# isaac-chandler/cuda-raytracer

Hardware: AMD Instinct MI355X
Metric: Mrays/s (live ray segments/s, teapot) (higher is better)
Workload: dtype f32

## Files before the change

cuda-raytracer_amd/csrc/rt_render.hip:

```cpp
#include "rt_common.h"

#include <algorithm>
#include <chrono>
#include <cstdio>
#include <cstdlib>
#include <cstring>
#include <string>
#include <thread>
#include <vector>

#include <rccl/rccl.h>

#pragma clang fp contract(off)

int rtamd_render_multi(const rt_scene *scene, const rt_opts *opts, float *fb_out, rt_stats *stats);

using namespace rtamd;

namespace {

#ifndef RT_INFLIGHT
#define RT_INFLIGHT 20
#endif
#ifndef RT_TRACE_OCC
// ... 20 lines not shown
    return (n + span - 1) / span;
}
inline int max_tiles(int64_t n_max) {
    return n_max >= (int64_t)kTileTarget * kSortTile ? (int)((n_max + kSortTile - 1) / kSortTile)
                                                    : (int)std::min<int64_t>(kTileTarget, (n_max + kBlock - 1) / kBlock);
}
inline int tile_stride(int64_t n_max) {
    return (int)std::max<int64_t>(kTileTarget, (n_max + kSortTile - 1) / kSortTile);
}
constexpr int kBuckets = 65;
constexpr int kInflight = RT_INFLIGHT;
constexpr int kStaggerUs = 4000;
constexpr int kStaggerGroup = 4;
constexpr int kStaggerMinPasses = 8;
constexpr int kStaggerShortUs = 2000;
constexpr int kTraceOccPct = RT_TRACE_OCC;
constexpr uint32_t kDead = 64;
constexpr uint32_t kAccFlag = 0x80000000u;
constexpr int kSpanSlots = 8;
constexpr int kSpanWords = 2 * kSpanSlots;
#ifdef RT_PROFILE
__device__ unsigned long long g_prof[2][14];
#define PROF(i, v) (prof[i] += (v))
#else
#define PROF(i, v) ((void)0)
#endif

struct FastDiv {
    uint32_t m = 0;
    int l = 0;
    static FastDiv of(uint32_t d) {
        FastDiv f;
        if (d > 1) {
            f.l = 32 - __builtin_clz(d - 1);
            f.m = (uint32_t)((((uint64_t)1 << (31 + f.l)) + d - 1) / d);
        }
        return f;
    }
    __device__ __forceinline__ uint32_t div(uint32_t n) const { return l == 0 ? n : (__umulhi(n, m) >> (l - 1)); }
};

struct SlotMap {
    FastDiv by_stripe;
    uint32_t skip, base;
    static SlotMap identity() { return SlotMap{FastDiv::of(0x7fffffffu), 0u, 0u}; }
    static SlotMap of(uint32_t stripe, int count, int index) {
        return SlotMap{FastDiv::of(stripe), (uint32_t)(count - 1) * stripe, (uint32_t)index * stripe};
    }
    __device__ __forceinline__ uint32_t ray(uint32_t s) const { return s + by_stripe.div(s) * skip + base; }
};

template <int FIRST>
__device__ __forceinline__ uint32_t first_ray(const SlotMap &m, uint32_t slot) {
    return FIRST == 2 ? m.ray(slot) : slot;
}

struct PassArgs {
    int rtc;
    uint32_t gen_seed_term;
    FastDiv by_rtc, by_width;
    SlotMap map;
};

__device__ __forceinline__ V3 primary_dir(const DevScene &S, int i, const PassArgs &pa) {
    Rng rng = pcg_seed((uint32_t)i * 0x85810BEAu + pa.gen_seed_term);
    uint32_t z;
    asm volatile("v_mov_b32 %0, 0" : "=v"(z));
    rng.inc += z;
    const uint32_t pixel = pa.by_rtc.div((uint32_t)i);
    const uint32_t yy = pa.by_width.div(pixel);
    const int x = (int)(pixel - yy * (uint32_t)S.width), y = (int)yy;
    const float xc = (x + random01(rng)) * S.inv_w;
    const float yc = (y + random01(rng)) * S.inv_h;
    return normalise(S.tl + xc * S.sr - yc * S.su);
}

#ifndef RT_FUSED_MAX_TRIS
#define RT_FUSED_MAX_TRIS 4096
#endif
#ifndef RT_SORT_GRID
#define RT_SORT_GRID 0
#endif

template <bool SORTED, bool COUNT, int FIRST>
__global__ __launch_bounds__(kBlock) RT_TRACE_ATTR void trace_kernel(DevScene S, PassArgs pa, const float4 *__restrict__ geo,
                                                       const uint32_t *__restrict__ live_count,
                                                       uint32_t *__restrict__ queue, float2 *__restrict__ hits,
                                                       uint32_t *__restrict__ overflow, Counters *__restrict__ ctr,
                                                       unsigned long long *__restrict__ tspan) {
    __shared__ uint2 stack[(kStackLds + 1) * kBlock];
    const unsigned long long t_start = wall_clock64();
    uint2 *col = stack + threadIdx.x;
    const uint32_t lanes = gridDim.x * kBlock, gl = blockIdx.x * kBlock + threadIdx.x;
    const uint32_t dist_half = lanes * (kStackMax - kStackLds);
    const uint32_t L = __builtin_amdgcn_readfirstlane(*live_count);
    const uint32_t waves = gridDim.x * (kBlock / 64);
    const uint32_t chunk = min((uint32_t)kChunkMax, max((uint32_t)kChunkMin, (L / (4 * waves) + 63) & ~63u));
    uint32_t shard = blockIdx.x % kQueues, tried = 0;
    uint32_t q_next = 0, q_end = 0;
    bool exhausted = false;
    int slot = -1;
    V3 o{0, 0, 0}, d{0, 0, 0};
    float ix = 0, iy = 0, iz = 0, closest = 0;
    bool finite_inv = true;
    bool wave_nonfinite = false;
    int index = -1, sp = 0;
    uint32_t ref = 0;
    int ti = 0, te = 0;
    unsigned pn = 0, iv = 0, tt = 0, nlive = 0;
#ifdef RT_PROFILE
    unsigned long long prof[14] = {0, 0, 0, 0, 0, 0, 0, 0, 0, 0, 0, 0, 0, 0};
#endif
    auto node_step = [&](float4 a, float4 b, float4 c, uint2 kids) -> bool {
        if (COUNT) iv++;
        float t0, t1;
        bool h0, h1;
        slab_pair(a, b, c, o, ix, iy, iz, closest, h0, h1, t0, t1);
        if (__builtin_expect(wave_nonfinite, 0)) {
            float u0, u1;
            const bool g0 = slab(a.x, a.z, b.x, b.z, c.x, c.z, o, ix, iy, iz, closest, u0);
            const bool g1 = slab(a.y, a.w, b.y, b.w, c.y, c.w, o, ix, iy, iz, closest, u1);
            if (!finite_inv) { h0 = g0; h1 = g1; t0 = u0; t1 = u1; }
        }
        const bool both = h0 && h1, any = h0 || h1;
        const bool sel1 = h1 && (!h0 || t0 < t1);
        const uint32_t next_ref = sel1 ? kids.y : kids.x, near_ref = sel1 ? kids.x : kids.y;
        const float next_t = sel1 ? t1 : t0, near_t = sel1 ? t0 : t1;
        col[min(sp, kStackLds) * kBlock] = make_uint2(near_ref, __float_as_uint(near_t));
        if (__builtin_expect(both && sp >= kStackLds, 0)) {
            overflow[(sp - kStackLds) * lanes + gl] = near_ref;
            overflow[dist_half + (sp - kStackLds) * lanes + gl] = __float_as_uint(near_t);
        }
        if (both) sp++;
        ref = any ? next_ref : ref;
        const bool descend = any && !(next_t >= closest);
        bool need = !descend;
        if (descend) {
            if (COUNT) pn++;
            if (ref & kLeaf) {
                leaf_range(S, ref, ti, te);
                need = ti == te;
            }
        }
        return need;
    };
    auto pop_loop = [&](bool need) {
        while (need) {
            PROF(10, 1);
            const bool empty = sp == 0;
            sp = empty ? 0 : sp - 1;
            uint2 e = col[min(sp, kStackLds) * kBlock];
            asm volatile("" : "+v"(e.x), "+v"(e.y));
            if (__builtin_expect(__ballot(sp >= kStackLds) != 0, 0)) {
                if (sp >= kStackLds) {
                    e.x = overflow[(sp - kStackLds) * lanes + gl];
                    e.y = overflow[dist_half + (sp - kStackLds) * lanes + gl];
                }
            }
            const bool take = !empty && !(__uint_as_float(e.y) >= closest);
            slot = empty ? -2 - slot : slot;
            ref = take ? e.x : ref;
            if (COUNT) pn += take ? 1u : 0u;
            const bool leaf = take && (ref & kLeaf);
            if (__builtin_expect(leaf && (ref & kBigLeaf), 0)) {
                leaf_range(S, ref, ti, te);
            } else {
                ti = leaf ? (int)(ref & 0xFFFFFFu) : ti;
                te = leaf ? ti + (int)((ref >> 24) & 0x3Fu) : te;
            }
            need = !empty && (!take || (leaf && ti == te));
        }
    };
    const bool root_internal = !(S.root_ref & kLeaf);
    float4 ra{0, 0, 0, 0}, rb{0, 0, 0, 0}, rc{0, 0, 0, 0};
    uint2 rk{0, 0};
    if (root_internal) {
        const float4 *rr = S.nodes + (size_t)S.root_ref * 4;
        const float4 x0 = rr[0], x1 = rr[1], x2 = rr[2];
        const uint2 k = *reinterpret_cast<const uint2 *>(rr + 3);
#define RT_U(v) __int_as_float(__builtin_amdgcn_readfirstlane(__float_as_int(v)))
        ra = make_float4(RT_U(x0.x), RT_U(x0.y), RT_U(x0.z), RT_U(x0.w));
        rb = make_float4(RT_U(x1.x), RT_U(x1.y), RT_U(x1.z), RT_U(x1.w));
        rc = make_float4(RT_U(x2.x), RT_U(x2.y), RT_U(x2.z), RT_U(x2.w));
#undef RT_U
        rk = make_uint2(__builtin_amdgcn_readfirstlane(k.x), __builtin_amdgcn_readfirstlane(k.y));
    }
    while (true) {
        unsigned long long idle = __ballot(slot < 0);
        if (!exhausted && __popcll(idle) >= (FIRST ? kRefillFirst : kRefill)) {
            PROF(6, 1);
            if (slot <= -2) {
                hits[-2 - slot] = make_float2(closest, __int_as_float(index));
                slot = -1;
            }
            bool fresh = false;
            while (idle && !exhausted) {
                if (q_next >= q_end) {
                    const uint32_t seg_lo = (uint32_t)(((uint64_t)L * shard) / kQueues);
                    const uint32_t seg_hi = (uint32_t)(((uint64_t)L * (shard + 1)) / kQueues);
                    uint32_t c = 0;
                    if (lane_id() == 0) c = atomicAdd(queue + shard * kQueueStride, chunk);
                    c = __builtin_amdgcn_readfirstlane(__shfl(c, 0)) + seg_lo;
                    if (c >= seg_hi) {
                        shard = (shard + 1) % kQueues;
                        if (++tried == kQueues) exhausted = true;
                        continue;
                    }
                    q_next = c;
                    q_end = min(c + chunk, seg_hi);
                }
                const uint32_t avail = q_end - q_next;
                const uint32_t r = rank_below(idle);
                const bool take = slot < 0 && r < avail;
                const unsigned long long took = __ballot(take);
                if (take) { slot = (int)(q_next + r); fresh = true; }
                q_next += (uint32_t)__popcll(took);
                idle &= ~took;
            }
            if (fresh) {
                {
                    nlive++;
                    if (FIRST) {
                        o = S.cam;
                        d = primary_dir(S, (int)first_ray<FIRST>(pa.map, (uint32_t)slot), pa);
                    } else {
                        const float4 *rp = geo + (size_t)slot * 2;
                        const float4 r0 = rp[0];
                        const float2 r1 = *reinterpret_cast<const float2 *>(rp + 1);
                        o = v3(r0.x, r0.y, r0.z);
                        d = v3(r0.w, r1.x, r1.y);
                    }
                    ix = 1 / d.x; iy = 1 / d.y; iz = 1 / d.z;
                    finite_inv = __builtin_isfinite(ix) && __builtin_isfinite(iy) && __builtin_isfinite(iz);

                    closest = 1e30f;
                    index = -1;
                    for (int i = 0; i < S.sphere_count; i++) {
                        const float4 sph = S.spheres[i];
                        float t;
                        if (ray_sphere(o, d, v3(sph.x, sph.y, sph.z), sph.w, closest, t)) { closest = t; index = i; }
                    }
                    ref = S.root_ref;
                    sp = 0;
                    if (COUNT) pn++;
                    ti = te = 0;
                    if (ref & kLeaf) {
                        leaf_range(S, ref, ti, te);
                        if (ti == te) {
                            hits[slot] = make_float2(closest, __int_as_float(index));
                            slot = -1;
                        }
                    }
                }
            }
            wave_nonfinite = __ballot(slot >= 0 && !finite_inv) != 0;
            if (root_internal && __ballot(fresh && slot >= 0)) {
                bool need = false;
                if (fresh && slot >= 0) need = node_step(ra, rb, rc, rk);
                pop_loop(need);
            }
        }
        if (!__ballot(slot >= 0)) {
            if (exhausted) break;
            PROF(7, 1);
            continue;
        }
#ifdef RT_PROFILE
        {
            const unsigned long long act = __ballot(slot >= 0), lf = __ballot(slot >= 0 && ti < te);
            PROF(0, 1); PROF(1, __popcll(act)); PROF(2, __popcll(lf));
            PROF(3, lf != 0); PROF(4, (act & ~lf) != 0);
            const bool mixed = lf != 0 && (act & ~lf) != 0;
            PROF(8, mixed);
            if (mixed) PROF(9, min(__popcll(lf), __popcll(act & ~lf)));
            const uintptr_t ra = slot >= 0 ? (uintptr_t)(ti < te ? S.tris + (size_t)ti * 3 : S.nodes + (size_t)ref * 4) : 0;
            const int first = __builtin_ctzll(act);
            const uintptr_t r0 = ((uintptr_t)__shfl((unsigned)(ra >> 32), first) << 32) | __shfl((unsigned)ra, first);
            const unsigned long long same = __ballot(slot >= 0 && ra == r0);
            PROF(12, same == act);
            PROF(13, 4 * __popcll(same) >= 3 * __popcll(act));
        }
#endif
        if (slot < 0) continue;
        bool need = false;
        const bool in_leaf = ti < te;
        const float4 *rec = in_leaf ? S.tris + (size_t)ti * 3 : S.nodes + (size_t)ref * 4;
        const float4 a = rec[0], b = rec[1], c = rec[2];
        uint2 kids = make_uint2(0, 0);
        if (!in_leaf) kids = *reinterpret_cast<const uint2 *>(rec + 3);
        if (in_leaf) {
            const float4 q0 = a, q1 = b;
            const float q2 = c.x;
            if (COUNT) tt++;
            float t;
            const bool hit =
                ray_triangle_flat(o, d, v3(q0.x, q0.y, q0.z), v3(q0.w, q1.x, q1.y), v3(q1.z, q1.w, q2), closest, t);
            closest = hit ? t : closest;
            index = hit ? S.sphere_count + ti : index;
            need = ++ti == te;
        } else {
            need = node_step(a, b, c, kids);
// ... 499 lines not shown
            if (threadIdx.x < kBuckets) {
                uint32_t s2 = 0;
                for (int k = 0; k < kBlock / 64; k++) { s2 += wcount[k][threadIdx.x]; wcount[k][threadIdx.x] = 0; }
                run[threadIdx.x] += s2;
            }
            __syncthreads();
        }
    }
}
__global__ void delay_kernel(unsigned long long ticks) {
    const unsigned long long t0 = wall_clock64();
    while (wall_clock64() - t0 < ticks) __builtin_amdgcn_s_sleep(127);
}

__global__ void set_count_kernel(uint32_t *__restrict__ dst, uint32_t v, const uint32_t *__restrict__ src) {
    if (threadIdx.x == 0) *dst = src ? *src : v;
}

template <bool SORTED, int FIRST, bool INLINE>
__global__ __launch_bounds__(kBlock) RT_REPLAY_ATTR void sort_scatter_shade_kernel(DevScene S, PassArgs pa,
                                                                    const uint8_t *__restrict__ bkt_in,
                                                                    const float4 *__restrict__ geo_in,
                                                                    const float *__restrict__ tz_in,
                                                                    const uint32_t *__restrict__ rid_in,
                                                                    const float2 *__restrict__ hits, uint32_t seed_term,
                                                                    const uint32_t *__restrict__ live_count, int tiles,
                                                                    const uint32_t *__restrict__ offsets,
                                                                    const uint32_t *__restrict__ totals,
                                                                    float4 *__restrict__ geo_out,
                                                                    float *__restrict__ tz_out,
                                                                    uint32_t *__restrict__ rid_out,
                                                                    float4 *__restrict__ acc = nullptr,
                                                                    uint32_t *__restrict__ home_of = nullptr,
                                                                    uint32_t home_base = 0) {
    const bool homes = FIRST == 1 && home_of != nullptr;
    const int n = (int)*live_count;
    __shared__ uint32_t run[kBuckets];
    __shared__ uint32_t wcount[kBlock / 64][kBuckets];
    const int R = tile_rounds(n), span = kBlock * R;
    for (int tile = blockIdx.x; tile * span < n; tile += gridDim.x) {
        bucket_runs(run, offsets, totals, tiles, tile);
        for (int k = threadIdx.x; k < (kBlock / 64) * kBuckets; k += kBlock) (&wcount[0][0])[k] = 0;
        __syncthreads();
        const int wave = threadIdx.x >> 6;
        const int base = tile * span;
        const int rounds = min(R, (n - base + kBlock - 1) / kBlock);
        for (int r = 0; r < rounds; r++) {
            const int item = base + r * kBlock + threadIdx.x;
            const bool valid = item < n;
            const uint32_t b = valid ? bkt_in[item] : 0u;
            const bool move = valid && b != kDead;
            Shaded sh{};
            if (move) sh = shade_one<SORTED, FIRST, INLINE>(S, pa, item, geo_in, tz_in, rid_in, hits, seed_term);
            const unsigned long long peers = match_bucket(b, valid);
            const uint32_t rank = rank_below(peers);
            if (valid && rank == 0) wcount[wave][b] = (uint32_t)__popcll(peers);
            __syncthreads();
            if (move) {
                uint32_t pos = run[b] + rank;
                for (int k = 0; k < wave; k++) pos += wcount[k][b];
                geo_out[(size_t)pos * 2] = make_float4(sh.no.x, sh.no.y, sh.no.z, sh.nd.x);
                geo_out[(size_t)pos * 2 + 1] = make_float4(sh.nd.y, sh.nd.z, sh.T.x, sh.T.y);
                tz_out[pos] = sh.T.z;
                const uint32_t id = homes ? home_base + pos : sh.ray;
                if (homes) {
                    home_of[item] = id;
                    if (has_radiance(sh.C)) acc[id] = make_float4(sh.T.z, sh.C.x, sh.C.y, sh.C.z);
                }
                rid_out[pos] = id | (has_radiance(sh.C) || sh.acc_holds ? kAccFlag : 0u);
            } else if (homes && valid) {
                home_of[item] = (uint32_t)item;
            }
            __syncthreads();
            if (threadIdx.x < kBuckets) {
                uint32_t s = 0;
                for (int k = 0; k < kBlock / 64; k++) { s += wcount[k][threadIdx.x]; wcount[k][threadIdx.x] = 0; }
                run[threadIdx.x] += s;
            }
            __syncthreads();
        }
    }
}

constexpr int kAccPixels = 64;
template <bool TILED>
__global__ __launch_bounds__(kBlock) void accumulate_kernel(const float4 *__restrict__ tc, int rtc, int pixels,
                                                            float *__restrict__ sums, SlotMap pix,
                                                            const uint32_t *__restrict__ home_of = nullptr) {
    __shared__ float col[kAccPixels * 20 * 3];
    const int p0 = blockIdx.x * kAccPixels;
    const int np = min(kAccPixels, pixels - p0);
    const int n = np * rtc;
    const float4 *src = tc + (size_t)p0 * rtc;
    for (int e = threadIdx.x; e < n; e += kBlock) {
        const float4 c = TILED     ? tc[(size_t)pix.ray((uint32_t)(p0 + e / rtc)) * rtc + e % rtc]
                         : home_of ? tc[home_of[(size_t)p0 * rtc + e]]
                                   : src[e];
        col[e * 3] = c.y;
        col[e * 3 + 1] = c.z;
        col[e * 3 + 2] = c.w;
    }
    __syncthreads();
    const int t = threadIdx.x;
    if (t >= np) return;
    float sx = 0, sy = 0, sz = 0;
    const float *r = col + t * rtc * 3;
    for (int s = 0; s < rtc; s++) {
        sx = sx + r[s * 3];
        sy = sy + r[s * 3 + 1];
        sz = sz + r[s * 3 + 2];
    }
    const size_t p = TILED ? (size_t)pix.ray((uint32_t)(p0 + t)) : (size_t)(p0 + t);
    sums[p * 3] = sx;
    sums[p * 3 + 1] = sy;
    sums[p * 3 + 2] = sz;
}

__global__ __launch_bounds__(kBlock) void high_pass_kernel(const float *__restrict__ img, float *__restrict__ out,
                                                           float threshold, int pixels) {
    const int i = blockIdx.x * kBlock + threadIdx.x;
    if (i >= pixels) return;
    const V3 c = v3(img[3 * i], img[3 * i + 1], img[3 * i + 2]);
    const bool bright = dot(c, v3(0.2126f, 0.7152f, 0.0722f)) > threshold;
    out[3 * i] = bright ? c.x : 0.0f;
    out[3 * i + 1] = bright ? c.y : 0.0f;
    out[3 * i + 2] = bright ? c.z : 0.0f;
}

template <bool VERTICAL>
__global__ __launch_bounds__(kBlock) void box_blur_kernel(const float *__restrict__ in, float *__restrict__ out,
                                                          int radius, int w, int h) {
    const int i = blockIdx.x * kBlock + threadIdx.x;
    if (i >= w * h) return;
    const int x = i % w, y = i / w;
    float sx = 0, sy = 0, sz = 0;
    int count = 0;
    for (int k = -radius; k <= radius; k++) {
        const int nx = VERTICAL ? x : x + k, ny = VERTICAL ? y + k : y;
        if (VERTICAL ? (ny >= 0 && ny < h) : (nx >= 0 && nx < w)) {
            const float *p = in + ((size_t)ny * w + nx) * 3;
            sx = sx + p[0];
            sy = sy + p[1];
            sz = sz + p[2];
            count++;
        }
    }
    const float k = 1.0f / count;
    out[3 * i] = k * sx;
    out[3 * i + 1] = k * sy;
    out[3 * i + 2] = k * sz;
}

__global__ __launch_bounds__(kBlock) void add_kernel(float *__restrict__ img, const float *__restrict__ add, int n) {
    const int i = blockIdx.x * kBlock + threadIdx.x;
    if (i < n) img[i] = img[i] + add[i];
}
__global__ __launch_bounds__(kBlock) void add4_kernel(float *__restrict__ img, const float *__restrict__ add, int n) {
    const int i = blockIdx.x * kBlock + threadIdx.x;
    const int n4 = n >> 2;
    if (i < n4) {
        float4 a = reinterpret_cast<float4 *>(img)[i];
        const float4 b = reinterpret_cast<const float4 *>(add)[i];
        a.x = a.x + b.x; a.y = a.y + b.y; a.z = a.z + b.z; a.w = a.w + b.w;
        reinterpret_cast<float4 *>(img)[i] = a;
    }
    if (i < (n & 3)) img[(n4 << 2) + i] = img[(n4 << 2) + i] + add[(n4 << 2) + i];
}

__attribute__((constructor(101))) void rtamd_default_hw_queues() {
    setenv("GPU_MAX_HW_QUEUES", "24", 0);
}
int queues_granted() {
    const char *q = std::getenv("GPU_MAX_HW_QUEUES");
    const int n = q ? std::atoi(q) : 0;
    return n > 0 ? n : 4;
}

}

int rtamd::trace_closest_blocks_per_cu(int &per_cu) {
    HIPCHK(hipOccupancyMaxActiveBlocksPerMultiprocessor(&per_cu, trace_kernel<false, false, 0>, kBlock, 0));
    return RT_OK;
}
void rtamd::launch_trace_closest(bool count, int grid, hipStream_t s, const DevScene &ds, const float4 *geo,
                                 const uint32_t *live, uint32_t *queue, float2 *hits, uint32_t *overflow, Counters *ctr) {
    const PassArgs pa{1, 0u, FastDiv::of(1), FastDiv::of((uint32_t)ds.width), SlotMap::identity()};
    if (count)
        hipLaunchKernelGGL((trace_kernel<false, true, 0>), dim3(grid), dim3(kBlock), 0, s, ds, pa, geo, live, queue, hits,
                           overflow, ctr, nullptr);
    else
        hipLaunchKernelGGL((trace_kernel<false, false, 0>), dim3(grid), dim3(kBlock), 0, s, ds, pa, geo, live, queue, hits,
                           overflow, ctr, nullptr);
}

struct InitTimer {
    std::chrono::high_resolution_clock::time_point t = std::chrono::high_resolution_clock::now();
    std::string out;
    bool on = std::getenv("RTAMD_TIMING") != nullptr;
    void mark(const char *what) {
        if (!on) return;
        const auto now = std::chrono::high_resolution_clock::now();
        char buf[96];
        std::snprintf(buf, sizeof(buf), " %s %.1f ms,", what, std::chrono::duration<double, std::milli>(now - t).count());
        out += buf;
        t = now;
    }
    void report() const { if (on) std::fprintf(stderr, "rt_renderer init:%s\n", out.c_str()); }
};

struct PassCtx {
    hipStream_t stream = nullptr;
    DevBuf<float4> geo[2], acc;
    DevBuf<float> tz[2];
    DevBuf<uint32_t> rid[2], sort_counts, sort_offsets, sort_totals, live, queue, overflow;
    DevBuf<uint8_t> bkt;
    DevBuf<float2> hits;
    DevBuf<uint32_t> home_of;
    DevBuf<float> psum;
    DevBuf<uint32_t> gslot[2], newpos, glive;
    DevBuf<uint8_t> gbytes, lbytes;
    uint32_t *lg_host = nullptr;
    hipEvent_t lg_ready = nullptr;
    int t_p = 0, t_k = 0, t_b = -1, t_rtc = 0, t_rem = 0, t_n = 0, t_cur = 0, t_tiles_g = 0;
    uint64_t t_lg = 0;
    hipEvent_t fb_done = nullptr;
    hipEvent_t done = nullptr;
    std::vector<hipEvent_t> events;
    size_t ev = 0;

    ~PassCtx() {
        if (lg_host) (void)hipHostFree(lg_host);
        if (lg_ready) (void)hipEventDestroy(lg_ready);
        for (auto e : events) (void)hipEventDestroy(e);
        if (fb_done) (void)hipEventDestroy(fb_done);
        if (done) (void)hipEventDestroy(done);
        if (stream) (void)hipStreamDestroy(stream);
    }
    int open() {
        if (stream) return RT_OK;
        HIPCHK(hipStreamCreateWithFlags(&stream, hipStreamNonBlocking));
        HIPCHK(hipEventCreateWithFlags(&fb_done, hipEventDisableTiming));
        HIPCHK(hipEventCreateWithFlags(&done, hipEventDisableTiming));
        return RT_OK;
    }
    hipEvent_t event() {
        if (ev == events.size()) {
            hipEvent_t e;
            if (hipEventCreate(&e) != hipSuccess) return nullptr;
            events.push_back(e);
        }
        return events[ev++];
    }
};

struct rt_renderer {
    bool sort = true, counters = false;
    int tile_count = 1, tile_index = 0, tile_rows = 8;
    bool pass_events = true;
    bool fused = false;
    bool inline_hits = false;
    int fused_upto = -1;
    bool home = false;
    uint32_t home_base = 0;
    int width = 0, height = 0, spp = 0, bounces = 0;
    SceneDev scene;
    DevBuf<float> fb;
    DevBuf<unsigned long long> tspans;
    int wall_khz = 0;
    std::vector<double> launch_ms;
    std::vector<uint32_t> launch_live;
    bool shade_hist = !std::getenv("RTAMD_SHADE_HIST") || std::atoi(std::getenv("RTAMD_SHADE_HIST")) != 0;
    int stagger_us = std::getenv("RTAMD_STAGGER_US") ? std::max(0, std::min(20000, std::atoi(std::getenv("RTAMD_STAGGER_US"))))
                                                    : kStaggerUs;
    int short_stagger_us = std::getenv("RTAMD_STAGGER_SHORT_US")
                               ? std::max(0, std::min(20000, std::atoi(std::getenv("RTAMD_STAGGER_SHORT_US")))) : kStaggerShortUs;
    PassCtx ctx[kInflight];
    int pass_hint = 0;
    int inflight_limit = 0;
    int trace_blocks = 0;
    int trace_blocks_max = 0;
    int nctx = 1;
    int inflight_cap = kInflight;
    hipEvent_t t_begin = nullptr, t_end = nullptr;

    ~rt_renderer() {
        (void)hipSetDevice(scene.device);
        if (run_pending && t_end) (void)hipEventSynchronize(t_end);
        for (hipEvent_t e : pass_done) (void)hipEventDestroy(e);
        if (xcomm) {
            (void)hipSetDevice(scene.device);
            if (failed) (void)ncclCommAbort(static_cast<ncclComm_t>(xcomm));
            for (auto &c : ctx)
                if (c.stream) (void)hipStreamSynchronize(c.stream);
            if (!failed) (void)ncclCommDestroy(static_cast<ncclComm_t>(xcomm));
        }
        if (xhost) (void)hipHostFree(xhost);
        if (t_begin) (void)hipEventDestroy(t_begin);
        if (t_end) (void)hipEventDestroy(t_end);
    }

    hipStream_t stream() const { return ctx[0].stream; }
    rt_exchange_fn xfn = nullptr;
    void *xuser = nullptr;
    bool x_on_device = false;
    uint8_t *xhost = nullptr;
    int (*xpoll)(void *) = nullptr;
    void *xpoll_user = nullptr;
    void *xcomm = nullptr;
    DevBuf<int32_t> sched;
    bool tsort() const { return tile_count > 1 && sort; }
    int pass_count() const { return (spp + 19) / 20; }
    bool tiled() const { return tile_count > 1; }
    int64_t tile_pixels() const {
        if (!tiled()) return (int64_t)width * height;
        int64_t rows = 0;
        for (int k = tile_index; (int64_t)k * tile_rows < height; k += tile_count)
            rows += std::min(tile_rows, height - k * tile_rows);
        return rows * width;
    }

    int init(const rt_scene *sc, const rt_opts *o) {
        scene.device = o->device;
        sort = o->sort != 0;
        counters = o->collect_counters != 0;
        tile_count = std::max(1, o->tile_count);
        tile_index = o->tile_index;
        tile_rows = o->tile_rows > 0 ? o->tile_rows : 8;
        fused = sc->triangle_count <= RT_FUSED_MAX_TRIS;
        fused_upto = fused ? -1 : 0;
        if (const char *f = std::getenv("RTAMD_FUSED")) {
            const int v = std::atoi(f);
            fused = v == 1;
            fused_upto = v >= 2 ? v - 2 : -1;
        }
        inline_hits = fused && sc->triangle_count == 0;
        if (const char *f = std::getenv("RTAMD_INLINE")) inline_hits = fused && std::atoi(f) != 0 && sc->triangle_count == 0;
        if (tsort()) {
            fused = false;
            fused_upto = -1;
            inline_hits = false;
        }
        width = sc->width;
        height = sc->height;
        spp = sc->ray_count;
        bounces = sc->bounces;
        InitTimer tm;
        HIPCHK(hipSetDevice(o->device));
        tm.mark("hipSetDevice");
        if (int rc0 = ctx[0].open()) return rc0;
        tm.mark("first stream");
        HIPCHK(hipEventCreate(&t_begin));
        HIPCHK(hipEventCreate(&t_end));
        hipStream_t s0 = stream();
        int rc;
        if ((rc = scene.init(sc, o->device, s0))) return rc;
        const int64_t pixels = (int64_t)width * height;
        const int64_t max_rays = pixels * std::min(20, std::max(1, spp));
        if (max_rays > 0x7fffffff / 3) return rtamd::fail(RT_E_INVALID, "image too large for 32-bit ray indices");
        if ((rc = fb.alloc((size_t)pixels * 3))) return rc;
        int per_cu = 0;
        tm.mark("scene upload");
        HIPCHK(hipOccupancyMaxActiveBlocksPerMultiprocessor(&per_cu, trace_kernel<true, false, false>, kBlock, 0));
        tm.mark("occupancy query");
        trace_blocks_max = std::max(1, scene.cus * std::max(1, per_cu));
        trace_blocks = trace_blocks_max;
        const int tiles = tile_stride(max_rays);
        home = sort && !tiled() && bounces >= 2 && (fused || fused_upto >= 0);
        if (const char *e = std::getenv("RTAMD_HOME")) home = home && std::atoi(e) != 0;
        home_base = (uint32_t)max_rays;
        const size_t ctx_bytes = (size_t)max_rays * (2 * (32 + 4 + 4) + 16 + 1 + 8 + (tsort() ? 2 * 4 + 4 + 2 : 0) +
                                                     (home ? 16 + 4 : 0)) +
                                 (size_t)trace_blocks_max * kBlock * 8 * (kStackMax - kStackLds) + ((size_t)1 << 20);
        size_t mem_free = 0, mem_total = 0;
        HIPCHK(hipMemGetInfo(&mem_free, &mem_total));
        size_t cap = kInflight;
        if (inflight_limit > 0) cap = std::min<size_t>(cap, (size_t)inflight_limit);
        if (const char *e = std::getenv("RTAMD_INFLIGHT")) cap = std::min<size_t>(cap, (size_t)std::max(1, std::atoi(e)));
        cap = std::min<size_t>(cap, (size_t)queues_granted());
        inflight_cap = (int)cap;
        if (pass_hint > 0) cap = std::min<size_t>(cap, (size_t)pass_hint);
        nctx = (int)std::min<size_t>({cap, (size_t)std::max(1, pass_count()),
                                                    std::max<size_t>(1, mem_free / 2 / ctx_bytes)});
        if (tsort() && (size_t)nctx < std::min<size_t>(cap, (size_t)std::max(1, pass_count())))
            return rtamd::fail(RT_E_OOM, "pixel tiles with sort on: device memory holds only " + std::to_string(nctx) +
                                             " passes in flight; set RTAMD_INFLIGHT to the same lower value on every owner");
        const int inflight = nctx;
        for (int k = 0; k < inflight; k++) {
            PassCtx &c = ctx[k];
            if ((rc = c.open())) return rc;
            for (int q = 0; q < 2; q++) {
                if ((rc = c.geo[q].alloc((size_t)max_rays * 2))) return rc;
                if ((rc = c.tz[q].alloc((size_t)max_rays))) return rc;
                if ((rc = c.rid[q].alloc((size_t)max_rays))) return rc;
            }
            if ((rc = c.bkt.alloc((size_t)max_rays))) return rc;
            if ((rc = c.acc.alloc((size_t)max_rays * (home ? 2 : 1)))) return rc;
            if (home && (rc = c.home_of.alloc((size_t)max_rays))) return rc;
            if ((rc = c.sort_counts.alloc((size_t)kBuckets * tiles))) return rc;
            if ((rc = c.sort_offsets.alloc((size_t)kBuckets * tiles))) return rc;
            if ((rc = c.sort_totals.alloc(kBuckets))) return rc;
            if ((rc = c.live.alloc((size_t)bounces + 1))) return rc;
            if ((rc = c.queue.alloc((size_t)(bounces + 1) * kQueues * kQueueStride))) return rc;
            if ((rc = c.hits.alloc((size_t)max_rays))) return rc;
            if ((rc = c.overflow.alloc((size_t)trace_blocks_max * kBlock * 2 * (kStackMax - kStackLds)))) return rc;
            if ((rc = c.psum.alloc((size_t)pixels * 3))) return rc;
            if (tsort()) {
                for (int q = 0; q < 2; q++)
                    if ((rc = c.gslot[q].alloc((size_t)max_rays))) return rc;
                if ((rc = c.newpos.alloc((size_t)max_rays)) || (rc = c.gbytes.alloc((size_t)max_rays)) ||
                    (rc = c.lbytes.alloc((size_t)max_rays)) || (rc = c.glive.alloc(3)))
                    return rc;
                HIPCHK(hipHostMalloc(reinterpret_cast<void **>(&c.lg_host), sizeof(uint32_t)));
                HIPCHK(hipEventCreateWithFlags(&c.lg_ready, hipEventDisableTiming));
            }
        }
        tm.mark("pass contexts");
        HIPCHK(hipMemsetAsync(fb.p, 0, fb.n * sizeof(float), s0));
        HIPCHK(hipStreamSynchronize(s0));
        tm.mark("sync");
        tm.report();
        return RT_OK;
    }

    int enqueue_pass(PassCtx &c, int p, float *sums, int64_t &sorted, unsigned long long *tspan) {
        const int before = spp - 20 * p;
        const int rtc = std::min(before, 20);
        const int remaining = before - rtc;
        const int64_t pixels = (int64_t)width * height;
        const int64_t tpix = tile_pixels();
        const int n = (int)(rtc * tpix);
        const int grid = blocks_for(n);
        const int tiles = tile_stride(n);
        const int tgrid = std::min(grid, trace_blocks);
        const int sgrid = std::min(grid, scene.cus * RT_SHADE_BPC);
        const int sort_grid = std::max(1, std::min(max_tiles(n), RT_SORT_GRID > 0 ? RT_SORT_GRID : scene.cus * 8));
        hipStream_t st = c.stream;
        int cur = 0;
        if (n == 0) {
            for (int k = 0; pass_events && k < 3 * bounces + 2 * (bounces - 1); k++) {
                hipEvent_t e = c.event();
                if (!e) return rtamd::fail(RT_E_HIP, "hipEventCreate failed");
                HIPCHK(hipEventRecord(e, st));
            }
            HIPCHK(hipMemsetAsync(sums, 0, (size_t)pixels * 3 * sizeof(float), st));
            return RT_OK;
        }
        hipLaunchKernelGGL(fill_live_kernel, dim3(1), dim3(256), 0, st, c.live.p, (uint32_t)n, bounces + 1, c.queue.p, tspan);
        const uint32_t stripe_px = (uint32_t)(tile_rows * width);
        const SlotMap pix = tiled() ? SlotMap::of(stripe_px, tile_count, tile_index) : SlotMap::identity();
        const SlotMap map = tiled() ? SlotMap::of(stripe_px * (uint32_t)rtc, tile_count, tile_index) : SlotMap::identity();
        const PassArgs pa{rtc, 709579u * (uint32_t)remaining, FastDiv::of((uint32_t)rtc), FastDiv::of((uint32_t)width),
                          map};
        for (int b = 0; b < bounces; b++) {
            const uint32_t seed_term = 279220567u * (uint32_t)(remaining * 20 + b);
            hipEvent_t e0 = nullptr, em = nullptr, e1 = nullptr;
            if (pass_events) {
                e0 = c.event(); em = c.event(); e1 = c.event();
                if (!e0 || !em || !e1) return rtamd::fail(RT_E_HIP, "hipEventCreate failed");
                HIPCHK(hipEventRecord(e0, st));
            }
            const uint32_t *lv = c.live.p + b;
            uint32_t *q = c.queue.p + (size_t)b * kQueues * kQueueStride;
            const bool last = b + 1 == bounces;
            uint32_t *hist = shade_hist && !last ? c.sort_counts.p : nullptr;
#define RT_PROCESS3(SORTED, COUNT, FIRST)                                                                         \
    do {                                                                                                         \
        if (!inline_hits)                                                                                        \
            hipLaunchKernelGGL((trace_kernel<SORTED, COUNT, FIRST>), dim3(tgrid), dim3(kBlock), 0, st, scene.ds, pa, \
                               c.geo[cur].p, lv, q, c.hits.p, c.overflow.p, scene.ctr.p,                         \
                               tspan ? tspan + kSpanWords * b : nullptr);                                        \
        if (em) HIPCHK(hipEventRecord(em, st));                                                                  \
        if (inline_hits)                                                                                         \
            hipLaunchKernelGGL((shade_kernel<SORTED, COUNT, FIRST, true, true>), dim3(sgrid), dim3(kBlock), 0, st,\
                               scene.ds, pa, c.geo[cur].p, c.tz[cur].p, c.rid[cur].p, c.acc.p, c.bkt.p, lv, c.hits.p, \
                               seed_term, (int)last, scene.ctr.p, nullptr, hist, tiles, (int)(home && b == 0));  \
        else if (fused || b <= fused_upto)                                                                       \
            hipLaunchKernelGGL((shade_kernel<SORTED, COUNT, FIRST, true, false>), dim3(sgrid), dim3(kBlock), 0, \
                               st, scene.ds, pa, c.geo[cur].p, c.tz[cur].p, c.rid[cur].p, c.acc.p, c.bkt.p, lv, c.hits.p, \
                               seed_term, (int)last, scene.ctr.p, nullptr, hist, tiles, (int)(home && b == 0));  \
        else                                                                                                     \
            hipLaunchKernelGGL((shade_kernel<SORTED, COUNT, FIRST, false, false>), dim3(sgrid), dim3(kBlock), 0, \
                               st, scene.ds, pa, c.geo[cur].p, c.tz[cur].p, c.rid[cur].p, c.acc.p, c.bkt.p, lv, c.hits.p, \
                               seed_term, (int)last, scene.ctr.p, nullptr, hist, tiles, (int)(home && b == 0));  \
    } while (0)
#define RT_PROCESS(SORTED, COUNT)                                                                                \
    do {                                                                                                         \
        if (b == 0) RT_PROCESS3(SORTED, COUNT, 1); else RT_PROCESS3(SORTED, COUNT, 0);                           \
    } while (0)
            if (sort) {
                if (counters) RT_PROCESS(true, true); else RT_PROCESS(true, false);
            } else {
                if (b == 0 && tiled()) {
                    if (counters) RT_PROCESS3(false, true, 2); else RT_PROCESS3(false, false, 2);
                } else if (counters) RT_PROCESS(false, true); else RT_PROCESS(false, false);
            }
#undef RT_PROCESS
#undef RT_PROCESS3
            HIPCHK(hipGetLastError());
            if (pass_events) HIPCHK(hipEventRecord(e1, st));
            if (b + 1 != bounces) {
                hipEvent_t s0 = nullptr, s1 = nullptr;
                if (pass_events) {
                    s0 = c.event(); s1 = c.event();
                    if (!s0 || !s1) return rtamd::fail(RT_E_HIP, "hipEventCreate failed");
                    HIPCHK(hipEventRecord(s0, st));
                }
                if (!hist)
                    hipLaunchKernelGGL(sort_hist_kernel, dim3(sort_grid), dim3(kBlock), 0, st, c.bkt.p, lv, tiles,
                                       c.sort_counts.p);
                hipLaunchKernelGGL(sort_scan_kernel, dim3(kBuckets), dim3(kBlock), 0, st, c.sort_counts.p, lv, tiles,
                                   c.sort_offsets.p, c.sort_totals.p, c.live.p + b + 1);
                if (fused || b <= fused_upto) {
#define RT_FSC2(SO, FI, IN)                                                                                      \
    hipLaunchKernelGGL((sort_scatter_shade_kernel<SO, FI, IN>), dim3(sort_grid), dim3(kBlock), 0, st, scene.ds, pa, \
                       c.bkt.p, c.geo[cur].p, c.tz[cur].p, c.rid[cur].p, c.hits.p, seed_term, lv, tiles,          \
                       c.sort_offsets.p, c.sort_totals.p, c.geo[1 - cur].p, c.tz[1 - cur].p, c.rid[1 - cur].p,    \
                       c.acc.p, home && b == 0 ? c.home_of.p : nullptr, home_base)
#define RT_FSC(SO, FI) do { if (inline_hits) RT_FSC2(SO, FI, true); else RT_FSC2(SO, FI, false); } while (0)
                    if (sort) {
                        if (b == 0) RT_FSC(true, 1); else RT_FSC(true, 0);
                    } else {
                        if (b == 0 && tiled()) RT_FSC(false, 2); else if (b == 0) RT_FSC(false, 1); else RT_FSC(false, 0);
                    }
#undef RT_FSC
#undef RT_FSC2
                } else if (b == 0 && tiled())
                    hipLaunchKernelGGL(sort_scatter_kernel<2>, dim3(sort_grid), dim3(kBlock), 0, st, c.bkt.p, c.geo[cur].p,
                                       c.tz[cur].p, c.rid[cur].p, lv, tiles, c.sort_offsets.p, c.sort_totals.p,
                                       c.geo[1 - cur].p, c.tz[1 - cur].p, c.rid[1 - cur].p, pa.map);
                else if (b == 0)
                    hipLaunchKernelGGL(sort_scatter_kernel<1>, dim3(sort_grid), dim3(kBlock), 0, st, c.bkt.p, c.geo[cur].p,
                                       c.tz[cur].p, c.rid[cur].p, lv, tiles, c.sort_offsets.p, c.sort_totals.p,
                                       c.geo[1 - cur].p, c.tz[1 - cur].p, c.rid[1 - cur].p, pa.map);
                else
                    hipLaunchKernelGGL(sort_scatter_kernel<0>, dim3(sort_grid), dim3(kBlock), 0, st, c.bkt.p, c.geo[cur].p,
                                       c.tz[cur].p, c.rid[cur].p, lv, tiles, c.sort_offsets.p, c.sort_totals.p,
                                       c.geo[1 - cur].p, c.tz[1 - cur].p, c.rid[1 - cur].p, pa.map);
                HIPCHK(hipGetLastError());
                if (pass_events) HIPCHK(hipEventRecord(s1, st));
                cur = 1 - cur;
                if (sort) sorted += n;
            }
        }
        if (bounces == 0) {
            HIPCHK(hipMemsetAsync(sums, 0, (size_t)pixels * 3 * sizeof(float), st));
        } else if (!tiled()) {
            hipLaunchKernelGGL(accumulate_kernel<false>, dim3((unsigned)((pixels + kAccPixels - 1) / kAccPixels)),
                               dim3(kBlock), 0, st, c.acc.p, rtc, (int)pixels, sums, pix, home ? c.home_of.p : nullptr);
        } else {
            HIPCHK(hipMemsetAsync(sums, 0, (size_t)pixels * 3 * sizeof(float), st));
            if (tpix > 0)
                hipLaunchKernelGGL(accumulate_kernel<true>, dim3((unsigned)((tpix + kAccPixels - 1) / kAccPixels)),
                                   dim3(kBlock), 0, st, c.acc.p, rtc, (int)tpix, sums, pix);
        }
        HIPCHK(hipGetLastError());
        return RT_OK;
    }

    int wait_event(hipEvent_t e) {
        if (!xpoll) {
            HIPCHK(hipEventSynchronize(e));
            return RT_OK;
        }
        for (;;) {
            const hipError_t q = hipEventQuery(e);
            if (q == hipSuccess) return RT_OK;
            if (q != hipErrorNotReady) return hip_fail(q, "hipEventQuery");
            if (int rc = xpoll(xpoll_user)) return rtamd::fail(rc, "tile exchange aborted: another device of the render failed");
            std::this_thread::yield();
        }
    }
    int tsort_begin(PassCtx &c, int p, int k) {
        const int before = spp - 20 * p;
        c.t_p = p;
        c.t_k = k;
        c.t_b = 0;
        c.t_rtc = std::min(before, 20);
        c.t_rem = before - c.t_rtc;
        c.t_n = (int)(c.t_rtc * tile_pixels());
        c.t_cur = 0;
        c.t_lg = (uint64_t)c.t_rtc * width * height;
        c.t_tiles_g = tile_stride((int64_t)c.t_lg);
        hipLaunchKernelGGL(fill_live_kernel, dim3(1), dim3(256), 0, c.stream, c.live.p, (uint32_t)c.t_n, bounces + 1,
                           c.queue.p, nullptr);
        hipLaunchKernelGGL(set_count_kernel, dim3(1), dim3(64), 0, c.stream, c.glive.p, (uint32_t)c.t_lg, nullptr);
        HIPCHK(hipGetLastError());
        return RT_OK;
    }
    PassArgs tsort_args(const PassCtx &c) const {
        const uint32_t stripe_px = (uint32_t)(tile_rows * width);
        return PassArgs{c.t_rtc, 709579u * (uint32_t)c.t_rem, FastDiv::of((uint32_t)c.t_rtc), FastDiv::of((uint32_t)width),
                        SlotMap::of(stripe_px * (uint32_t)c.t_rtc, tile_count, tile_index)};
    }
    int tsort_front(PassCtx &c, int b, int64_t &sorted) {
        hipStream_t st = c.stream;
        const PassArgs pa = tsort_args(c);
        const int grid = blocks_for(c.t_n);
        const int tgrid = std::max(1, std::min(grid, trace_blocks));
        const int sgrid = std::max(1, std::min(grid, scene.cus * RT_SHADE_BPC));
        const uint32_t seed_term = 279220567u * (uint32_t)(c.t_rem * 20 + b);
        const uint32_t *lv = c.live.p + b;
        uint32_t *q = c.queue.p + (size_t)b * kQueues * kQueueStride;
        const int last = b + 1 == bounces;
        const int cur = c.t_cur;
        if (!last) {
            const int zgrid = std::max(1, std::min(blocks_for((int64_t)(c.t_lg + 15) / 16), scene.cus * 8));
            hipLaunchKernelGGL(zero_bytes_kernel, dim3(zgrid), dim3(kBlock), 0, st, c.gbytes.p, c.lbytes.p, c.glive.p);
        }
        if (c.t_n == 0) return RT_OK;
#define RT_TS(COUNT)                                                                                           \
    do {                                                                                                           \
        if (b == 0) {                                                                                              \
            hipLaunchKernelGGL((trace_kernel<true, COUNT, 2>), dim3(tgrid), dim3(kBlock), 0, st, scene.ds, pa,           \
                               c.geo[cur].p, lv, q, c.hits.p, c.overflow.p, scene.ctr.p, nullptr);                       \
            hipLaunchKernelGGL((shade_kernel<true, COUNT, 2, false, false>), dim3(sgrid), dim3(kBlock), 0, st, scene.ds, \
                               pa, c.geo[cur].p, c.tz[cur].p, c.rid[cur].p, c.acc.p, c.bkt.p, lv, c.hits.p,         \
                               seed_term, last, scene.ctr.p, nullptr);                                                   \
        } else {                                                                                                   \
            hipLaunchKernelGGL((trace_kernel<true, COUNT, 0>), dim3(tgrid), dim3(kBlock), 0, st, scene.ds, pa,           \
                               c.geo[cur].p, lv, q, c.hits.p, c.overflow.p, scene.ctr.p, nullptr);                       \
            hipLaunchKernelGGL((shade_kernel<true, COUNT, 0, false, false>), dim3(sgrid), dim3(kBlock), 0, st, scene.ds, \
                               pa, c.geo[cur].p, c.tz[cur].p, c.rid[cur].p, c.acc.p, c.bkt.p, lv, c.hits.p,         \
                               seed_term, last, scene.ctr.p, c.gslot[cur].p);                                            \
// ... 714 lines not shown
```

Measured before the change: 13790.

## Virtually reorder bounce-0 rays instead of scattering them, fusing rank with shade

For sorted non-tiled renders with two or more bounces, bounce 0 no longer scatters ray data into sorted order. Bounce 1's trace kernel reads rays through the bucket ranks directly and skips dead slots using a per-slot bucket byte. A new shade_rank_kernel then shades and scatters live rays into bucket order in one pass. A fill kernel pre-marks the next bucket array as dead. This removes a full scatter pass over ray state, at the cost of less coherent trace reads in bounce 1, an extra byte array, and a dead-slot retry loop in the queue refill.

```diff
diff --git a/cuda-raytracer_amd/csrc/rt_render.hip b/cuda-raytracer_amd/csrc/rt_render.hip
--- a/cuda-raytracer_amd/csrc/rt_render.hip
+++ b/cuda-raytracer_amd/csrc/rt_render.hip
@@ -126,12 +126,13 @@
 #define RT_SORT_GRID 0
 #endif
 
-template <bool SORTED, bool COUNT, int FIRST>
+template <bool SORTED, bool COUNT, int FIRST, bool VSLOT = false>
 __global__ __launch_bounds__(kBlock) RT_TRACE_ATTR void trace_kernel(DevScene S, PassArgs pa, const float4 *__restrict__ geo,
                                                        const uint32_t *__restrict__ live_count,
                                                        uint32_t *__restrict__ queue, float2 *__restrict__ hits,
                                                        uint32_t *__restrict__ overflow, Counters *__restrict__ ctr,
-                                                       unsigned long long *__restrict__ tspan) {
+                                                       unsigned long long *__restrict__ tspan,
+                                                       const uint8_t *__restrict__ slot_bkt = nullptr) {
     __shared__ uint2 stack[(kStackLds + 1) * kBlock];
     const unsigned long long t_start = wall_clock64();
     uint2 *col = stack + threadIdx.x;
@@ -238,29 +239,36 @@
                 slot = -1;
             }
             bool fresh = false;
-            while (idle && !exhausted) {
-                if (q_next >= q_end) {
-                    const uint32_t seg_lo = (uint32_t)(((uint64_t)L * shard) / kQueues);
-                    const uint32_t seg_hi = (uint32_t)(((uint64_t)L * (shard + 1)) / kQueues);
-                    uint32_t c = 0;
-                    if (lane_id() == 0) c = atomicAdd(queue + shard * kQueueStride, chunk);
-                    c = __builtin_amdgcn_readfirstlane(__shfl(c, 0)) + seg_lo;
-                    if (c >= seg_hi) {
-                        shard = (shard + 1) % kQueues;
-                        if (++tried == kQueues) exhausted = true;
-                        continue;
+            do {
+                bool got = false;
+                while (idle && !exhausted) {
+                    if (q_next >= q_end) {
+                        const uint32_t seg_lo = (uint32_t)(((uint64_t)L * shard) / kQueues);
+                        const uint32_t seg_hi = (uint32_t)(((uint64_t)L * (shard + 1)) / kQueues);
+                        uint32_t c = 0;
+                        if (lane_id() == 0) c = atomicAdd(queue + shard * kQueueStride, chunk);
+                        c = __builtin_amdgcn_readfirstlane(__shfl(c, 0)) + seg_lo;
+                        if (c >= seg_hi) {
+                            shard = (shard + 1) % kQueues;
+                            if (++tried == kQueues) exhausted = true;
+                            continue;
+                        }
+                        q_next = c;
+                        q_end = min(c + chunk, seg_hi);
                     }
-                    q_next = c;
-                    q_end = min(c + chunk, seg_hi);
+                    const uint32_t avail = q_end - q_next;
+                    const uint32_t r = rank_below(idle);
+                    const bool take = slot < 0 && r < avail;
+                    const unsigned long long took = __ballot(take);
+                    if (take) { slot = (int)(q_next + r); fresh = true; got = true; }
+                    q_next += (uint32_t)__popcll(took);
+                    idle &= ~took;
                 }
-                const uint32_t avail = q_end - q_next;
-                const uint32_t r = rank_below(idle);
-                const bool take = slot < 0 && r < avail;
-                const unsigned long long took = __ballot(take);
-                if (take) { slot = (int)(q_next + r); fresh = true; }
-                q_next += (uint32_t)__popcll(took);
-                idle &= ~took;
-            }
+                if (VSLOT) {
+                    if (got && slot_bkt[slot] == kDead) { slot = -1; fresh = false; }
+                    idle = __ballot(slot < 0);
+                }
+            } while (VSLOT && idle && !exhausted);
             if (fresh) {
                 {
                     nlive++;
@@ -926,6 +934,103 @@
     }
 }
 
+
+__global__ __launch_bounds__(kBlock) void fill_dead_kernel(uint8_t *__restrict__ bkt, const uint32_t *__restrict__ count) {
+    const uint32_t n = *count;
+    const uint32_t n16 = n / 16;
+    const uint32_t w = kDead * 0x01010101u;
+    for (uint32_t i = blockIdx.x * kBlock + threadIdx.x; i < n16; i += gridDim.x * kBlock)
+        reinterpret_cast<uint4 *>(bkt)[i] = make_uint4(w, w, w, w);
+    for (uint32_t i = n16 * 16 + blockIdx.x * kBlock + threadIdx.x; i < n; i += gridDim.x * kBlock) bkt[i] = (uint8_t)kDead;
+}
+
+template <bool COUNT>
+__global__ __launch_bounds__(kBlock) RT_SHADE_ATTR void shade_rank_kernel(DevScene S, PassArgs pa,
+                                                            const uint8_t *__restrict__ bkt_in,
+                                                            const float4 *__restrict__ geo_in,
+                                                            const float *__restrict__ tz_in,
+                                                            const uint32_t *__restrict__ rid_in,
+                                                            const float2 *__restrict__ hits, uint32_t seed_term, int last,
+                                                            const uint32_t *__restrict__ slot_count, int tiles,
+                                                            const uint32_t *__restrict__ offsets,
+                                                            const uint32_t *__restrict__ totals,
+                                                            float4 *__restrict__ geo_out, float *__restrict__ tz_out,
+                                                            uint32_t *__restrict__ rid_out, uint8_t *__restrict__ bkt_out,
+                                                            float4 *__restrict__ acc, Counters *__restrict__ ctr) {
+    const int n = (int)__builtin_amdgcn_readfirstlane(*slot_count);
+    __shared__ uint32_t run[kBuckets];
+    __shared__ uint32_t wcount[kBlock / 64][kBuckets];
+    unsigned hit = 0, miss = 0, hit_sphere = 0;
+    const int R = tile_rounds(n), span = kBlock * R;
+    for (int tile = blockIdx.x; tile * span < n; tile += gridDim.x) {
+        bucket_runs(run, offsets, totals, tiles, tile);
+        for (int k = threadIdx.x; k < (kBlock / 64) * kBuckets; k += kBlock) (&wcount[0][0])[k] = 0;
+        __syncthreads();
+        const int wave = threadIdx.x >> 6;
+        const int base = tile * span;
+        const int rounds = min(R, (n - base + kBlock - 1) / kBlock);
+        for (int r = 0; r < rounds; r++) {
+            const int item = base + r * kBlock + threadIdx.x;
+            const bool valid = item < n;
+            const uint32_t b = valid ? bkt_in[item] : 0u;
+            const bool move = valid && b != kDead;
+            ShadeIn in{};
+            if (move) in = shade_in<true, 0, false>(pa, item, geo_in, tz_in, rid_in, hits, nullptr);
+            const unsigned long long peers = match_bucket(b, valid);
+            const uint32_t rank = rank_below(peers);
+            if (valid && rank == 0) wcount[wave][b] = (uint32_t)__popcll(peers);
+            __syncthreads();
+            if (move) {
+                uint32_t pos = run[b] + rank;
+                for (int k = 0; k < wave; k++) pos += wcount[k][b];
+                in.seed = pos;
+                const Shaded sh = shade_from<true, 0>(S, pa, item, in, seed_term);
+                const V3 no = sh.no, nd = sh.nd, T = sh.T;
+                miss += sh.kind == 0;
+                hit += sh.kind != 0;
+                hit_sphere += sh.kind == 2;
+                const bool dead = is_black(T);
+                const bool term = has_radiance(sh.C);
+                if (dead || last || term) {
+                    V3 C = sh.C;
+                    if (sh.acc_holds) {
+                        const float4 a = acc[sh.ray];
+                        C = v3(a.y, a.z, a.w) + sh.C;
+                    }
+                    typedef float f4v __attribute__((ext_vector_type(4)));
+                    if (dead || last)
+                        __builtin_nontemporal_store(f4v{T.z, C.x, C.y, C.z}, reinterpret_cast<f4v *>(acc + sh.ray));
+                    else
+                        acc[sh.ray] = make_float4(T.z, C.x, C.y, C.z);
+                }
+                if (!dead && !last) {
+                    geo_out[(size_t)pos * 2] = make_float4(no.x, no.y, no.z, nd.x);
+                    geo_out[(size_t)pos * 2 + 1] = make_float4(nd.y, nd.z, T.x, T.y);
+                    tz_out[pos] = T.z;
+                    rid_out[pos] = sh.ray | (term || sh.acc_holds ? kAccFlag : 0u);
+                    bkt_out[pos] = (uint8_t)bucket_of(no, nd, S.min_coord, S.inv_dim);
+                }
+            }
+            __syncthreads();
+            if (threadIdx.x < kBuckets) {
+                uint32_t s = 0;
+                for (int k = 0; k < kBlock / 64; k++) { s += wcount[k][threadIdx.x]; wcount[k][threadIdx.x] = 0; }
+                run[threadIdx.x] += s;
+            }
+            __syncthreads();
+        }
+    }
+    if (COUNT) {
+        Counters *cs = ctr + ((blockIdx.x * (kBlock / 64) + (threadIdx.x >> 6)) & (kCtrSlots - 1));
+        const unsigned long long h = wave_sum(hit), m = wave_sum(miss), hs = wave_sum(hit_sphere);
+        if (lane_id() == 0 && (h | m)) {
+            atomicAdd(&cs->hits, h);
+            atomicAdd(&cs->misses, m);
+            atomicAdd(&cs->hits_sphere, hs);
+        }
+    }
+}
+
 constexpr int kAccPixels = 64;
 template <bool TILED>
 __global__ __launch_bounds__(kBlock) void accumulate_kernel(const float4 *__restrict__ tc, int rtc, int pixels,
@@ -1058,6 +1163,7 @@
     DevBuf<float> tz[2];
     DevBuf<uint32_t> rid[2], sort_counts, sort_offsets, sort_totals, live, queue, overflow;
     DevBuf<uint8_t> bkt;
+    DevBuf<uint8_t> bkt1;
     DevBuf<float2> hits;
     DevBuf<uint32_t> home_of;
     DevBuf<float> psum;
@@ -1106,6 +1212,7 @@
     int fused_upto = -1;
     bool home = false;
     uint32_t home_base = 0;
+    bool vre = false;
     int width = 0, height = 0, spp = 0, bounces = 0;
     SceneDev scene;
     DevBuf<float> fb;
@@ -1209,11 +1316,14 @@
         trace_blocks_max = std::max(1, scene.cus * std::max(1, per_cu));
         trace_blocks = trace_blocks_max;
         const int tiles = tile_stride(max_rays);
-        home = sort && !tiled() && bounces >= 2 && (fused || fused_upto >= 0);
+        const bool vre_can = sort && !tiled() && bounces >= 2 && sc->triangle_count > 0;
+        vre = vre_can && !std::getenv("RTAMD_FUSED") && !fused && fused_upto == 0;
+        if (const char *e = std::getenv("RTAMD_VREORDER")) vre = vre_can && std::atoi(e) != 0;
+        home = !vre && sort && !tiled() && bounces >= 2 && (fused || fused_upto >= 0);
         if (const char *e = std::getenv("RTAMD_HOME")) home = home && std::atoi(e) != 0;
         home_base = (uint32_t)max_rays;
         const size_t ctx_bytes = (size_t)max_rays * (2 * (32 + 4 + 4) + 16 + 1 + 8 + (tsort() ? 2 * 4 + 4 + 2 : 0) +
-                                                     (home ? 16 + 4 : 0)) +
+                                                     (home ? 16 + 4 : 0) + (vre ? 1 : 0)) +
                                  (size_t)trace_blocks_max * kBlock * 8 * (kStackMax - kStackLds) + ((size_t)1 << 20);
         size_t mem_free = 0, mem_total = 0;
         HIPCHK(hipMemGetInfo(&mem_free, &mem_total));
@@ -1238,6 +1348,7 @@
                 if ((rc = c.rid[q].alloc((size_t)max_rays))) return rc;
             }
             if ((rc = c.bkt.alloc((size_t)max_rays))) return rc;
+            if (vre && (rc = c.bkt1.alloc((size_t)max_rays))) return rc;
             if ((rc = c.acc.alloc((size_t)max_rays * (home ? 2 : 1)))) return rc;
             if (home && (rc = c.home_of.alloc((size_t)max_rays))) return rc;
             if ((rc = c.sort_counts.alloc((size_t)kBuckets * tiles))) return rc;
@@ -1262,6 +1373,7 @@
         HIPCHK(hipMemsetAsync(fb.p, 0, fb.n * sizeof(float), s0));
         HIPCHK(hipStreamSynchronize(s0));
         tm.mark("sync");
+        if (tm.on) tm.out += vre ? " bounce-0 reorder: virtual" : " bounce-0 reorder: moved";
         tm.report();
         return RT_OK;
     }
@@ -1306,8 +1418,10 @@
             const uint32_t *lv = c.live.p + b;
             uint32_t *q = c.queue.p + (size_t)b * kQueues * kQueueStride;
             const bool last = b + 1 == bounces;
-            uint32_t *hist = shade_hist && !last ? c.sort_counts.p : nullptr;
-#define RT_PROCESS3(SORTED, COUNT, FIRST)                                                                         \
+            const bool v0 = vre && b == 0, v1 = vre && b == 1;
+            const bool fuse_b = !v0 && !v1 && (fused || b <= fused_upto);
+            uint32_t *hist = shade_hist && !last && !v1 ? c.sort_counts.p : nullptr;
+#define RT_PROCESS3(SORTED, COUNT, FIRST)                                                                        \
     do {                                                                                                         \
         if (!inline_hits)                                                                                        \
             hipLaunchKernelGGL((trace_kernel<SORTED, COUNT, FIRST>), dim3(tgrid), dim3(kBlock), 0, st, scene.ds, pa, \
@@ -1318,7 +1432,7 @@
             hipLaunchKernelGGL((shade_kernel<SORTED, COUNT, FIRST, true, true>), dim3(sgrid), dim3(kBlock), 0, st,\
                                scene.ds, pa, c.geo[cur].p, c.tz[cur].p, c.rid[cur].p, c.acc.p, c.bkt.p, lv, c.hits.p, \
                                seed_term, (int)last, scene.ctr.p, nullptr, hist, tiles, (int)(home && b == 0));  \
-        else if (fused || b <= fused_upto)                                                                       \
+        else if (fuse_b)                                                                                         \
             hipLaunchKernelGGL((shade_kernel<SORTED, COUNT, FIRST, true, false>), dim3(sgrid), dim3(kBlock), 0, \
                                st, scene.ds, pa, c.geo[cur].p, c.tz[cur].p, c.rid[cur].p, c.acc.p, c.bkt.p, lv, c.hits.p, \
                                seed_term, (int)last, scene.ctr.p, nullptr, hist, tiles, (int)(home && b == 0));  \
@@ -1331,7 +1445,22 @@
     do {                                                                                                         \
         if (b == 0) RT_PROCESS3(SORTED, COUNT, 1); else RT_PROCESS3(SORTED, COUNT, 0);                           \
     } while (0)
-            if (sort) {
+            if (v1) {
+#define RT_VPROCESS(COUNT)                                                                                       \
+    do {                                                                                                         \
+        hipLaunchKernelGGL((trace_kernel<true, COUNT, 0, true>), dim3(tgrid), dim3(kBlock), 0, st, scene.ds, pa, \
+                           c.geo[cur].p, c.live.p, q, c.hits.p, c.overflow.p, scene.ctr.p,                       \
+                           tspan ? tspan + kSpanWords * b : nullptr, c.bkt.p);                                   \
+        if (em) HIPCHK(hipEventRecord(em, st));                                                                  \
+        hipLaunchKernelGGL((shade_rank_kernel<COUNT>), dim3(sort_grid), dim3(kBlock), 0, st, scene.ds, pa, c.bkt.p, \
+                           c.geo[cur].p, c.tz[cur].p, c.rid[cur].p, c.hits.p, seed_term, (int)last, c.live.p, tiles, \
+                           c.sort_offsets.p, c.sort_totals.p, c.geo[1 - cur].p, c.tz[1 - cur].p, c.rid[1 - cur].p, \
+                           c.bkt1.p, c.acc.p, scene.ctr.p);                                                      \
+    } while (0)
+                if (counters) RT_VPROCESS(true); else RT_VPROCESS(false);
+#undef RT_VPROCESS
+                cur = 1 - cur;
+            } else if (sort) {
                 if (counters) RT_PROCESS(true, true); else RT_PROCESS(true, false);
             } else {
                 if (b == 0 && tiled()) {
@@ -1349,12 +1478,16 @@
                     if (!s0 || !s1) return rtamd::fail(RT_E_HIP, "hipEventCreate failed");
                     HIPCHK(hipEventRecord(s0, st));
                 }
+                const uint8_t *bk = v1 ? c.bkt1.p : c.bkt.p;
                 if (!hist)
-                    hipLaunchKernelGGL(sort_hist_kernel, dim3(sort_grid), dim3(kBlock), 0, st, c.bkt.p, lv, tiles,
+                    hipLaunchKernelGGL(sort_hist_kernel, dim3(sort_grid), dim3(kBlock), 0, st, bk, lv, tiles,
                                        c.sort_counts.p);
                 hipLaunchKernelGGL(sort_scan_kernel, dim3(kBuckets), dim3(kBlock), 0, st, c.sort_counts.p, lv, tiles,
                                    c.sort_offsets.p, c.sort_totals.p, c.live.p + b + 1);
-                if (fused || b <= fused_upto) {
+                if (v0) {
+                    if (b + 2 != bounces)
+                        hipLaunchKernelGGL(fill_dead_kernel, dim3(sort_grid), dim3(kBlock), 0, st, c.bkt1.p, c.live.p + 1);
+                } else if (fuse_b) {
 #define RT_FSC2(SO, FI, IN)                                                                                      \
     hipLaunchKernelGGL((sort_scatter_shade_kernel<SO, FI, IN>), dim3(sort_grid), dim3(kBlock), 0, st, scene.ds, pa, \
                        c.bkt.p, c.geo[cur].p, c.tz[cur].p, c.rid[cur].p, c.hits.p, seed_term, lv, tiles,          \
@@ -1377,12 +1510,12 @@
                                        c.tz[cur].p, c.rid[cur].p, lv, tiles, c.sort_offsets.p, c.sort_totals.p,
                                        c.geo[1 - cur].p, c.tz[1 - cur].p, c.rid[1 - cur].p, pa.map);
                 else
-                    hipLaunchKernelGGL(sort_scatter_kernel<0>, dim3(sort_grid), dim3(kBlock), 0, st, c.bkt.p, c.geo[cur].p,
+                    hipLaunchKernelGGL(sort_scatter_kernel<0>, dim3(sort_grid), dim3(kBlock), 0, st, bk, c.geo[cur].p,
                                        c.tz[cur].p, c.rid[cur].p, lv, tiles, c.sort_offsets.p, c.sort_totals.p,
                                        c.geo[1 - cur].p, c.tz[1 - cur].p, c.rid[1 - cur].p, pa.map);
                 HIPCHK(hipGetLastError());
                 if (pass_events) HIPCHK(hipEventRecord(s1, st));
-                cur = 1 - cur;
+                if (!v0) cur = 1 - cur;
                 if (sort) sorted += n;
             }
         }
```

New measurement: 14400, median of 6. +4.5%, better.
